# helgeanl/GP-MPC

Measured on NVIDIA H100. Metric: GP predictions/sec (N train x horizon test, fp64), higher is better.
Workload: dtype f64

## Files before the change

gp-mpc_b200/csrc/gpmpc.cu:

```cuda
#include "../../include/gpmpc.h"

#include <dlfcn.h>
#include <math.h>
#include <stdarg.h>
#include <stdlib.h>
#include <string.h>

#include <algorithm>
#include <array>
#include <functional>
#include <map>
#include <memory>
#include <type_traits>
#include <vector>

#include <nvtx3/nvToolsExt.h>

#include "common.cuh"
#include "gemm_dmma.cuh"
#include "predict_streamk.cuh"
#include "kernels.cuh"

#define GPMPC_VERSION 100
#define HB 64
// ... 948 lines not shown
    int used = 0;
    rc = factor_entries(h, e, 1, 1e-8, &used);
    if (rc) return rc;
    if (used > 1) { set_error(h, "gpmpc_loo_nlpp: K not positive definite even with jitter"); return GPMPC_ERR_NOTPD; }
    rc = alpha_pass(h, e);
    if (rc) return rc;
    LooLayout o;
    rc = loo_layout(h, 1, &o);
    if (rc) return rc;
    rc = loo_launch(h, al, 1, o, grad != nullptr);
    if (rc) return rc;
    double val = 0.0;
    CUDA_TRY(cudaMemcpyAsync(&val, o.nlpp, 8, cudaMemcpyDeviceToHost, h->st));
    if (grad) {
        rc = compute_kinv(h, al);
        if (rc) return rc;
        trmv_lower_kernel<<<(N + 7) / 8, 256, 0, h->st>>>(e.Li, np, 0, o.u, 0, o.tmp, 0, N);
        CUDA_TRY(cudaGetLastError());
        trmv_lower_T_kernel<<<(N + 31) / 32, 256, 0, h->st>>>(e.Li, np, 0, o.tmp, 0, o.b, 0, N);
        CUDA_TRY(cudaGetLastError());
        loo_mirror_scale_kernel<<<dim3(np / 32, np / 32), dim3(32, 8), 0, h->st>>>(h->dKinv, np, o.sw, h->dU, N);
        CUDA_TRY(cudaGetLastError());
        GemmParams p;
        memset(&p, 0, sizeof(p));
        p.A = h->dU; p.lda = np; p.B = h->dU; p.ldb = np; p.C = h->dKinv; p.ldc = np;
        p.mt = np / 128; p.nt = np / 128; p.K = np; p.alpha = 1.0; p.beta = 0.0; p.lower = 1;
        CUDA_TRY(gemm128(h, h->st, true, p, 1, 1));
        loo_w_kernel<<<dim3((N + 255) / 256, N), 256, 0, h->st>>>(h->dKinv, np, o.b, e.alpha, N);
        CUDA_TRY(cudaGetLastError());
        CUDA_TRY(cudaMemsetAsync(o.zero, 0, (size_t)np * 8, h->st));
        rc = launch_grad_at(h, e.hyp, h->dKinv, o.zero, h->dGradPart, h->dGrad, 1);
        if (rc) return rc;
        CUDA_TRY(cudaMemcpyAsync(grad, h->dGrad, m * 8, cudaMemcpyDeviceToHost, h->st));
    }
    CUDA_TRY(cudaStreamSynchronize(h->st));
    if (grad)
        for (int q = 0; q < m; ++q) grad[q] *= 2.0;
    *nlpp = val;
    return GPMPC_OK;
}

extern "C" int gpmpc_get(gpmpc_handle_t h, int what, int a, double* dst)
{
    if (!h || !dst) return GPMPC_ERR_ARG;
    CUDA_TRY(cudaSetDevice(h->device));
    const int al = local_index(h, a);
    if (al < 0) return GPMPC_ERR_ARG;
    if (what == GPMPC_GET_K) return gpmpc_build_K(h, a, dst);
    if (what != GPMPC_GET_ALPHA_NLML) {
        const int rc = model_guard(h, __func__, NEED_FACTOR);
        if (rc) return rc;
    }
    switch (what) {
    case GPMPC_GET_CHOL: return extract_to_host(h, h->dL + (long long)al * slab(h), dst, 1);
    case GPMPC_GET_LINV: return extract_to_host(h, h->dLi + (long long)al * slab(h), dst, 1);
    case GPMPC_GET_ALPHA:
    case GPMPC_GET_ALPHA_NLML:
        CUDA_TRY(cudaMemcpyAsync(dst, h->dAlpha + (long long)al * h->Npad, h->N * 8, cudaMemcpyDeviceToHost, h->st));
        CUDA_TRY(cudaStreamSynchronize(h->st));
        return GPMPC_OK;
    case GPMPC_GET_LOGDET: dst[0] = h->logdet[al]; return GPMPC_OK;
    case GPMPC_GET_INVK: {
        int rc = compute_kinv(h, al);
        if (rc) return rc;
        return extract_to_host(h, h->dKinv, dst, 2);
    }
    default: set_error(h, "gpmpc_get: unknown selector %d", what); return GPMPC_ERR_ARG;
    }
}

extern "C" int gpmpc_set_option(gpmpc_handle_t h, const char* name, double value)
{
    if (!h || !name) return GPMPC_ERR_ARG;
    if (!strcmp(name, "refine")) { h->opt_refine = value != 0.0; return GPMPC_OK; }
    if (!strcmp(name, "predict_ctas")) {
        const int v = (int)value;
        if (v < 0 || v > PSK_MAX_CTAS) { set_error(h, "predict_ctas must be in [0, %d]", PSK_MAX_CTAS); return GPMPC_ERR_ARG; }
        h->opt_predict_ctas = v; return GPMPC_OK;
    }
    if (!strcmp(name, "peer_timeout_s")) { h->opt_peer_timeout_s = value > 0.0 ? value : 60.0; return GPMPC_OK; }
    if (!strcmp(name, "small_tiles")) { h->opt_small_tiles = (int)value; return GPMPC_OK; }
    if (!strcmp(name, "peer")) { h->opt_peer = value != 0.0; return GPMPC_OK; }
    if (!strcmp(name, "em_points")) {
        if (!(value >= 0.0 && value <= 1e9)) { set_error(h, "em_points must be >= 0"); return GPMPC_ERR_ARG; }
        h->opt_em_points = (int)value; return GPMPC_OK;
    }
    if (!strcmp(name, "nlml_batch_max")) {
        if (!(value >= 0.0 && value <= 1e9)) { set_error(h, "nlml_batch_max must be >= 0"); return GPMPC_ERR_ARG; }
        h->opt_nlml_batch_max = (int)value; return GPMPC_OK;
    }
    set_error(h, "unknown option %s", name);
    return GPMPC_ERR_ARG;
}

static inline int ks_chunk(gpmpc_handle_t h)
{
    if (h->Npad < 8192) return 128;
    return (h->nloc >= 2 && h->Nx <= 12) ? 1024 : 512;
}

static inline int ks_blocks(gpmpc_handle_t h) { return (h->Npad + ks_chunk(h) - 1) / ks_chunk(h); }

static inline int round8(int n) { return (n + 7) / 8 * 8; }

static int ensure_rows(gpmpc_handle_t h)
{
    ENSURE(h->dV, (long long)h->nloc * HB * h->Npad);
    ENSURE(h->dR, (long long)h->nloc * HB * h->Npad);
    return GPMPC_OK;
}

static int ensure_predict_bufs(gpmpc_handle_t h, int H)
{
    const long long np = h->Npad, nt = np / 128;
    ENSURE(h->dKST, (long long)h->nloc * HB * np);
    ENSURE(h->dPMJ, (long long)h->nloc * HB * ks_blocks(h) * (h->Nx + 1));
    ENSURE(h->dSQ, (long long)h->nloc * HB * nt);
    ENSURE(h->dCnt, (long long)h->nloc * nt + h->nloc + 1);
    ENSURE(h->dPart, (long long)std::max(h->psk_ctas, h->opt_predict_ctas) * 2 * HB * PSK_BN);
    if (h->opt_refine) {
        int rc = ensure_rows(h);
        if (rc) return rc;
        ENSURE(h->dR2, (long long)h->nloc * HB * np);
    }
    if (H > h->Hcap) {
        h->Hcap = 0;
        h->dZ = h->dSigma = h->dMean = h->dVar = h->dJ = h->dCov = nullptr;
        const long long cap = std::max(H, HB);
        const int nyp = h->nloc_max * h->world;
        const long long Nx = h->Nx, Ny = h->Ny;
        ENSURE(h->dG, (long long)nyp * cap * (Nx + 2));
        ENSURE(h->dIn, cap * Nx + cap * Nx * Nx);
        ENSURE(h->dOut, cap * (2 * Ny + Ny * Nx + Ny * Ny));
        h->dZ = h->dIn; h->dSigma = h->dIn + cap * Nx;
        h->dMean = h->dOut; h->dVar = h->dOut + cap * Ny; h->dJ = h->dOut + 2 * cap * Ny;
        h->dCov = h->dOut + 2 * cap * Ny + cap * Ny * Nx;
        h->Hcap = (int)cap;
    }
    return GPMPC_OK;
}

template <int BM>
static cudaError_t psk_launch_bm(const PredictParams& p, const double* A, long long sA, const double* B, long long sB,
                                 int np, int grid, cudaStream_t st)
{
    constexpr int BYTES = psk_pipe_doubles(BM) * 8 + 2 * PSK_STAGES * 8 + 1024;
    const cudaError_t e = smem_opt_in<predict_streamk_kernel<BM>>(BYTES);
    if (e != cudaSuccess) return e;
    CUtensorMap tmA, tmB;
    if (!tmap_make(&tmA, A, np, BM, np, sA, p.nloc, BM)) return cudaErrorInvalidValue;
    if (!tmap_make(&tmB, B, np, np, np, sB, p.nloc, PSK_BN)) return cudaErrorInvalidValue;
    cudaLaunchConfig_t cfg;
    memset(&cfg, 0, sizeof(cfg));
    cfg.gridDim = dim3(grid); cfg.blockDim = dim3(PSK_THREADS); cfg.dynamicSmemBytes = BYTES; cfg.stream = st;
    cudaLaunchAttribute attr[1];
    attr[0].id = cudaLaunchAttributeProgrammaticStreamSerialization;
    attr[0].val.programmaticStreamSerializationAllowed = 1;
    cfg.attrs = attr; cfg.numAttrs = 1;
    return cudaLaunchKernelEx(&cfg, predict_streamk_kernel<BM>, p, tmA, tmB);
}

static int psk_grid(gpmpc_handle_t h, long long G)
{
    int ctas = h->opt_predict_ctas > 0 ? h->opt_predict_ctas : h->psk_ctas;
    ctas = std::min(ctas, PSK_MAX_CTAS);
    const long long by_work = std::max(1LL, G / 4);
    return (int)std::min<long long>(ctas, h->opt_predict_ctas > 0 ? G : by_work);
}

static int psk_schedule(gpmpc_handle_t h, PredictParams& p, const double* B)
{
    int grid = psk_grid(h, p.G);
    if (B == h->dLi.p && !p.upper) {
        p.Lp = h->dLiP;
        p.upo = psk_pair_units(p.nloc, p.ntb, grid);
        if (p.upo && h->opt_predict_ctas == 0) grid = psk_pair_grid((long long)p.nloc * p.upo, grid);
    }
    return grid;
}

static cudaError_t psk_launch(gpmpc_handle_t h, const PredictParams& p0, const double* A, const double* B)
{
    const long long sA = (long long)HB * h->Npad, sB = slab(h);
    const int np = h->Npad;
    PredictParams p = p0;
    const int grid = psk_schedule(h, p, B);
    if (p.Lp)
        for (int a = 0; a < h->nloc; ++a)
            if (h->panel_row[a] < np) return cudaErrorIllegalState;
    switch (round8(p.Hc)) {
    case 8: return psk_launch_bm<8>(p, A, sA, B, sB, np, grid, h->st);
    case 16: return psk_launch_bm<16>(p, A, sA, B, sB, np, grid, h->st);
    case 24: return psk_launch_bm<24>(p, A, sA, B, sB, np, grid, h->st);
    case 32: return psk_launch_bm<32>(p, A, sA, B, sB, np, grid, h->st);
    case 40: return psk_launch_bm<40>(p, A, sA, B, sB, np, grid, h->st);
    case 48: return psk_launch_bm<48>(p, A, sA, B, sB, np, grid, h->st);
    case 56: return psk_launch_bm<56>(p, A, sA, B, sB, np, grid, h->st);
    default: return psk_launch_bm<64>(p, A, sA, B, sB, np, grid, h->st);
    }
}

static void psk_base(gpmpc_handle_t h, PredictParams& p, int Hc, int upper = 0)
{
    memset(&p, 0, sizeof(p));
    const long long nt = h->Npad / 128;
    p.nloc = h->nloc; p.nt = (int)nt; p.Hc = Hc; p.upper = upper;
    p.ntb = (int)((h->Npad + PSK_BN - 1) / PSK_BN); p.nk = h->Npad / GEMM_BK;
    p.T = psk_steps_per_output(p.ntb, p.nk, upper); p.G = p.T * h->nloc;
    p.part = h->dPart;
    p.tile_cnt = h->dCnt; p.out_cnt = h->dCnt + (long long)h->nloc * nt; p.done_cnt = p.out_cnt + h->nloc;
    p.SQ = h->dSQ;
    p.hyp = h->dHyp; p.hyp_ld = h->Nx + 2; p.Nx = h->Nx;
}

static int panel_refresh(gpmpc_handle_t h)
{
    PredictParams p;
    psk_base(h, p, HB);
    const long long blk = PSK_BN * GEMM_BK;
    const double* old = h->dLiP;
    ENSURE(h->dLiP, p.G * blk);
    if (h->dLiP.p != old) panel_stale(h, -1, 0);
    for (int a = 0; a < h->nloc; ++a) {
        if (h->panel_row[a] >= h->Npad) continue;
        const int jt0 = h->panel_row[a] / PSK_BN;
        panel_pack_kernel<<<dim3(p.nk, p.ntb - jt0), 256, 0, h->st>>>(h->dLi + a * slab(h), h->Npad, h->dLiP + a * p.T * blk,
                                                                      p.ntb, jt0);
        CUDA_TRY(cudaGetLastError());
        h->panel_row[a] = h->Npad;
    }
    return GPMPC_OK;
}

static void psk_finalize(gpmpc_handle_t h, PredictParams& p, int H, int h0)
{
    p.finalize = 1; p.PMJ = h->dPMJ; p.nblk_mj = ks_blocks(h);
    p.Gloc = h->dG; p.slot0 = h->a0; p.Htot = H; p.h0 = h0;
}

static AssembleArgs assemble_args(gpmpc_handle_t h, int H, int method, const double* Sigma, int spp,
                                  double* mean, double* var, double* J, double* cov)
{
    AssembleArgs as;
    memset(&as, 0, sizeof(as));
    as.G = h->dG; as.Ny = h->Ny; as.Nx = h->Nx; as.H = H; as.method_ta = (method == GPMPC_METHOD_TA);
    as.Sigma = Sigma; as.sigma_per_point = spp;
    as.mean = mean; as.var = var; as.J = J; as.cov = cov;
    as.world = 1;
    as.stage_g = (assemble_rows_doubles(H, h->Ny, h->Nx) <= psk_pipe_doubles(round8(std::min(H, HB)))) ? 1 : 0;
    return as;
}

template <int NXP, int CH>
static cudaError_t launch_ks(gpmpc_handle_t h, const double* dZc, int Hc)
{
    const int smem = (NXP + 1) * CH * 8, nblk = ks_blocks(h);
    const cudaError_t e = smem_opt_in<ks_tile_kernel<NXP, CH>>(smem);
    if (e != cudaSuccess) return e;
    dim3 g(nblk, round8(Hc) / 8, h->nloc);
    ks_tile_kernel<NXP, CH><<<g, 256, smem, h->st>>>(h->dXT, h->Npad, h->N, h->Nx, h->dHyp, h->Nx + 2, h->dAlpha, h->Npad,
                                                     dZc, Hc, h->dKST, h->Npad, (long long)HB * h->Npad, h->dPMJ, nblk);
    return cudaGetLastError();
}

template <int CH>
static cudaError_t launch_ks_nx(gpmpc_handle_t h, const double* dZc, int Hc)
{
    const int Nx = h->Nx;
    if (Nx <= 4) return launch_ks<4, CH>(h, dZc, Hc);
    if (Nx <= 6) return launch_ks<6, CH>(h, dZc, Hc);
    if (Nx <= 8) return launch_ks<8, CH>(h, dZc, Hc);
    if (Nx <= 10) return launch_ks<10, CH>(h, dZc, Hc);
    if (Nx <= 12) return launch_ks<12, CH>(h, dZc, Hc);
    if (CH <= 512) {
        if (Nx <= 16) return launch_ks<16, (CH <= 512 ? CH : 512)>(h, dZc, Hc);
        if (Nx <= 24) return launch_ks<24, (CH <= 512 ? CH : 512)>(h, dZc, Hc);
        return launch_ks<32, (CH <= 512 ? CH : 512)>(h, dZc, Hc);
    }
    return cudaErrorInvalidValue;
}

static cudaError_t launch_ks(gpmpc_handle_t h, const double* dZc, int Hc)
{
    switch (ks_chunk(h)) {
    case 1024: return launch_ks_nx<1024>(h, dZc, Hc);
    case 512: return launch_ks_nx<512>(h, dZc, Hc);
    default: return launch_ks_nx<128>(h, dZc, Hc);
    }
}

static int tri_product(gpmpc_handle_t h, const double* Amat, const double* T, int Hc, double* Vout)
{
    PredictParams p;
    psk_base(h, p, Hc);
    p.Vout = Vout; p.sV = (long long)HB * h->Npad; p.ldv = h->Npad;
    CUDA_TRY(psk_launch(h, p, Amat, T));
    return GPMPC_OK;
}

__global__ void axpby_rows_kernel(const double* __restrict__ x, const double* __restrict__ y, double a, double b,
                                  double* __restrict__ out, long long rowlen, long long srow, int rows)
{
    const long long i = (long long)blockIdx.x * blockDim.x + threadIdx.x;
    const int r = blockIdx.y, bz = blockIdx.z;
    if (i >= rowlen || r >= rows) return;
    const long long o = (long long)bz * srow + (long long)r * rowlen + i;
    out[o] = a * x[o] + b * y[o];
// ... 2106 lines not shown
```

gp-mpc_b200/csrc/predict_streamk.cuh:

```cuda
#pragma once
#include "common.cuh"
#include "gemm_dmma.cuh"

#define GPMPC_MAXW 16
#define PSK_CW 8
#define PSK_BN (32 * PSK_CW)
#define PSK_STAGES 5
#define PSK_CTAS_PER_SM 1
#define PSK_THREADS (32 * PSK_CW)

__host__ __device__ constexpr long long psk_pipe_doubles(int bm) { return (long long)PSK_STAGES * (bm + PSK_BN) * GEMM_BK; }


struct PeerArgs {
    double* base[GPMPC_MAXW];
    int world, rank;
    long long goff;
    int flag_idx;
    unsigned long long step;
    long long timeout_clocks;
};

struct AssembleArgs {
    const double* G;
    int Ny, Nx, H, method_ta;
    const double* Sigma; int sigma_per_point;
    double *mean, *var, *J, *cov;
    const unsigned long long* flags;
    int world; unsigned long long step; int* status;
    long long timeout_clocks;
    unsigned long long* dbg;
    int stage_g;
};

struct PredictParams {
    int nloc, nt, Hc;
    int ntb, nk;
    int upper;
    const double* Lp;
    long long T, G;
    int upo;
    double* part;
    unsigned int* tile_cnt;
    unsigned int* out_cnt;
    unsigned int* done_cnt;
    double* SQ;
    double* Vout; long long sV; int ldv;
    int finalize;
    const double* PMJ; int nblk_mj;
    const double* hyp; int hyp_ld, Nx;
    double* Gloc; int slot0, Htot, h0;
    PeerArgs pa; int use_peers, publish;
    AssembleArgs as; int do_assemble;
    unsigned long long* dbg;
};

__device__ __forceinline__ void tail_stamp(unsigned long long* dbg, int k, int tid)
{
    if (dbg && tid == 0) { unsigned long long t; asm volatile("mov.u64 %0, %%globaltimer;" : "=l"(t)); dbg[k] = t; }
}

template <bool WARP>
__device__ __forceinline__ void assemble_point(const AssembleArgs& A, int h, double* sh, int tid, int nth)
{
    const int Ny = A.Ny, Nx = A.Nx, H = A.H;
    double* Jh = sh; double* JS = sh + Ny * Nx; double* vh = sh + 2 * Ny * Nx;
    for (int idx = tid; idx < Ny * Nx; idx += nth) {
        const int a = idx / Nx, d = idx % Nx;
        const double v = __ldcg(A.G + (((long long)a) * H + h) * (Nx + 2) + 2 + d);
        Jh[idx] = v;
        if (A.J) A.J[((long long)h * Ny + a) * Nx + d] = v;
    }
    for (int a = tid; a < Ny; a += nth) {
        const double* g = A.G + (((long long)a) * H + h) * (Nx + 2);
        const double m = __ldcg(g), v = __ldcg(g + 1);
        if (A.mean) A.mean[(long long)h * Ny + a] = m;
        if (A.var) A.var[(long long)h * Ny + a] = v;
        vh[a] = v;
    }
    if (WARP) __syncwarp(); else __syncthreads();
    if (A.cov) {
        if (A.method_ta) {
            const double* Sg = A.Sigma + (A.sigma_per_point ? (long long)h * Nx * Nx : 0);
            for (int idx = tid; idx < Ny * Nx; idx += nth) {
                const int a = idx / Nx, e = idx % Nx;
                double s = 0.0;
                for (int d = 0; d < Nx; ++d) s = fma(Jh[a * Nx + d], Sg[d * Nx + e], s);
                JS[idx] = s;
            }
            if (WARP) __syncwarp(); else __syncthreads();
        }
        for (int idx = tid; idx < Ny * Ny; idx += nth) {
            const int a = idx / Ny, b = idx % Ny;
            double s = (a == b) ? vh[a] : 0.0;
            if (A.method_ta) {
                double t = 0.0;
                for (int e = 0; e < Nx; ++e) t = fma(JS[a * Nx + e], Jh[b * Nx + e], t);
                s += t;
            }
            A.cov[((long long)h * Ny + a) * Ny + b] = s;
        }
    }
    if (WARP) __syncwarp(); else __syncthreads();
}

__device__ __forceinline__ void assemble_flat_global(const AssembleArgs& A, double* JS, int tid, int nth)
{
    const int Ny = A.Ny, Nx = A.Nx, H = A.H, NyNx = Ny * Nx;
    const bool ta = A.cov && A.method_ta;
    for (int idx = tid; idx < H * NyNx; idx += nth) {
        const int h = idx / NyNx, r = idx - h * NyNx, a = r / Nx, e = r - a * Nx;
        const double* g = A.G + (((long long)a) * H + h) * (Nx + 2) + 2;
        if (A.J) A.J[idx] = __ldcg(g + e);
        if (ta) {
            const double* Sg = A.Sigma + (A.sigma_per_point ? (long long)h * Nx * Nx : 0);
            double s = 0.0;
            for (int d = 0; d < Nx; ++d) s = fma(__ldcg(g + d), Sg[d * Nx + e], s);
            JS[idx] = s;
        }
    }
    for (int idx = tid; idx < H * Ny; idx += nth) {
        const int h = idx / Ny, a = idx - h * Ny;
        const double* g = A.G + (((long long)a) * H + h) * (Nx + 2);
        if (A.mean) A.mean[idx] = __ldcg(g);
        if (A.var) A.var[idx] = __ldcg(g + 1);
    }
    __syncthreads();
    if (A.cov) {
        for (int idx = tid; idx < H * Ny * Ny; idx += nth) {
            const int h = idx / (Ny * Ny), r = idx - h * Ny * Ny, a = r / Ny, b = r - a * Ny;
            double s = (a == b) ? __ldcg(A.G + (((long long)a) * H + h) * (Nx + 2) + 1) : 0.0;
            if (ta) {
                const double* gb = A.G + (((long long)b) * H + h) * (Nx + 2) + 2;
                const double* js = JS + (h * Ny + a) * Nx;
                double t = 0.0;
                for (int e = 0; e < Nx; ++e) t = fma(js[e], __ldcg(gb + e), t);
                s += t;
            }
            A.cov[idx] = s;
        }
    }
}

__host__ __device__ inline long long assemble_rows_doubles(int H, int Ny, int Nx)
{
    return (long long)H * Ny * (((Nx + 2) | 1) + (Nx | 1)) + (long long)Nx * Nx;
}

__device__ __forceinline__ void assemble_rows(const AssembleArgs& A, double* sh, int tid, int nth)
{
    const int Ny = A.Ny, Nx = A.Nx, H = A.H, F = Nx + 2, FP = F | 1, NP = Nx | 1, R = H * Ny;
    const bool ta = A.cov && A.method_ta;
    double* Gs = sh;
    double* JS = Gs + R * FP;
    double* Ss = JS + R * NP;
    const bool sig_s = ta && !A.sigma_per_point;
    {
        const int tot = R * F, HF = H * F;
        if (sig_s) for (int i = tid; i < Nx * Nx; i += nth) Ss[i] = A.Sigma[i];
        constexpr int SB = 20;
        for (int idx = tid; idx < tot; idx += SB * nth) {
            double v[SB];
#pragma unroll
            for (int k = 0; k < SB; ++k) v[k] = (idx + k * nth < tot) ? __ldcg(A.G + idx + k * nth) : 0.0;
#pragma unroll
            for (int k = 0; k < SB; ++k) {
                const int o = idx + k * nth;
                if (o < tot) {
                    const int a = o / HF, rem = o - a * HF, h = rem / F, q = rem - h * F;
                    Gs[(h * Ny + a) * FP + q] = v[k];
                }
            }
        }
        __syncthreads();
    }
    tail_stamp(A.dbg, 3, tid);
    if (A.J) for (int i = tid; i < R * Nx; i += nth) { const int row = i / Nx; A.J[i] = Gs[row * FP + 2 + (i - row * Nx)]; }
    for (int idx = tid; idx < R; idx += nth) {
        const double* g = Gs + idx * FP;
        if (A.mean) A.mean[idx] = g[0];
        if (A.var) A.var[idx] = g[1];
        if (ta) {
            const int h = idx / Ny;
            const double* Sg = sig_s ? Ss : A.Sigma + (long long)h * Nx * Nx;
            for (int e0 = 0; e0 < Nx; e0 += 8) {
                double acc[8];
#pragma unroll
                for (int k = 0; k < 8; ++k) acc[k] = 0.0;
                for (int d = 0; d < Nx; ++d) {
                    const double jd = g[2 + d];
#pragma unroll
                    for (int k = 0; k < 8; ++k) if (e0 + k < Nx) acc[k] = fma(jd, Sg[d * Nx + e0 + k], acc[k]);
                }
#pragma unroll
                for (int k = 0; k < 8; ++k) if (e0 + k < Nx) JS[idx * NP + e0 + k] = acc[k];
            }
        }
    }
    __syncthreads();
    tail_stamp(A.dbg, 4, tid);
    if (A.cov) {
        const bool via_smem = Ny <= 8 && Ny <= NP;
        for (int idx = tid; idx < R; idx += nth) {
            const int h = idx / Ny, a = idx - h * Ny;
            const double var = Gs[idx * FP + 1];
            for (int b0 = 0; b0 < Ny; b0 += 8) {
                double acc[8];
#pragma unroll
                for (int k = 0; k < 8; ++k) acc[k] = 0.0;
                if (ta) {
                    for (int e = 0; e < Nx; ++e) {
                        const double je = JS[idx * NP + e];
#pragma unroll
                        for (int k = 0; k < 8; ++k) if (b0 + k < Ny) acc[k] = fma(je, Gs[(h * Ny + b0 + k) * FP + 2 + e], acc[k]);
                    }
                }
#pragma unroll
                for (int k = 0; k < 8; ++k) {
                    if (b0 + k < Ny) {
                        const double c = ((a == b0 + k) ? var : 0.0) + acc[k];
                        if (via_smem) JS[idx * NP + k] = c; else A.cov[(long long)idx * Ny + b0 + k] = c;
                    }
                }
            }
        }
        if (via_smem) {
            __syncthreads();
            for (int i = tid; i < R * Ny; i += nth) { const int row = i / Ny; A.cov[i] = JS[row * NP + (i - row * Ny)]; }
        }
    }
}

__device__ __forceinline__ void assemble_flat(const AssembleArgs& A, double* sh, int tid, int nth)
{
    if (A.stage_g) assemble_rows(A, sh, tid, nth);
    else assemble_flat_global(A, sh, tid, nth);
}

__device__ __forceinline__ bool peer_acquire(const AssembleArgs& A, int tid, int* sh_ok)
{
    if (!A.flags) return true;
    if (tid == 0) *sh_ok = 1;
    __syncthreads();
    if (tid < A.world) {
        const long long t0 = clock64();
        unsigned long long v;
        do {
            asm volatile("ld.acquire.sys.global.u64 %0, [%1];" : "=l"(v) : "l"(A.flags + tid) : "memory");
            if (v >= A.step) break;
            if (clock64() - t0 > A.timeout_clocks) {
                *reinterpret_cast<volatile int*>(A.status) = 1 + tid;
                *reinterpret_cast<volatile int*>(sh_ok) = 0;
                break;
            }
            __nanosleep(64);
        } while (true);
    }
    __syncthreads();
    return *reinterpret_cast<volatile int*>(sh_ok) != 0;
}

__global__ void __launch_bounds__(128)
assemble_kernel(const AssembleArgs A)
{
    extern __shared__ double sh[];
    __shared__ int ok;
    if (!peer_acquire(A, threadIdx.x, &ok)) return;
    for (int h = blockIdx.x; h < A.H; h += gridDim.x) assemble_point<false>(A, h, sh, threadIdx.x, blockDim.x);
}

#define PSK_SB (PSK_BN / GEMM_BK)
__host__ __device__ inline long long psk_kstart(int ntb, int nk, int upper, int jt)
{
    const long long full = (long long)(PSK_SB / 2) * jt * (jt + 1), d = (long long)PSK_SB * ntb - nk;
    return upper ? full - jt * d : (jt == ntb ? full - d : full);
}
__host__ __device__ inline long long psk_steps_per_output(int ntb, int nk, int upper) { return psk_kstart(ntb, nk, upper, ntb); }
__device__ __forceinline__ long long psk_kstart(const PredictParams& p, int jt) { return psk_kstart(p.ntb, p.nk, p.upper, jt); }
__host__ __device__ inline int psk_ksteps(int ntb, int nk, int upper, int jt)
{
    return upper ? nk - PSK_SB * (ntb - 1 - jt) : (PSK_SB * (jt + 1) < nk ? PSK_SB * (jt + 1) : nk);
}
__device__ __forceinline__ int psk_ksteps(const PredictParams& p, int jt) { return psk_ksteps(p.ntb, p.nk, p.upper, jt); }

__host__ __device__ inline int psk_pair_units(int nloc, int ntb, int grid)
{
    const long long upo = (ntb + 1) / 2, units = nloc * upo, rounds = (units + grid - 1) / grid;
    return (units >= grid && 8 * units >= 7 * rounds * grid) ? (int)upo : 0;
}
__host__ __device__ inline int psk_pair_grid(long long units, int grid)
{
    const long long rounds = (units + grid - 1) / grid;
    return (int)((units + rounds - 1) / rounds);
}
__host__ __device__ inline int psk_unit_steps(int ntb, int nk, int pu)
{
    const int jl = ntb - 1 - pu;
    return psk_ksteps(ntb, nk, 0, jl) + (pu != jl ? psk_ksteps(ntb, nk, 0, pu) : 0);
}
__host__ __device__ inline long long psk_pair_cta_steps(int nloc, int ntb, int nk, int upo, long long c, long long C)
{
    long long n = 0;
    for (long long u = c; u < (long long)nloc * upo; u += C) n += psk_unit_steps(ntb, nk, (int)(u % upo));
    return n;
}
__host__ __device__ inline void psk_pair_first(int ntb, int upo, long long u, int& a, int& jt)
{
    a = (int)(u / upo);
    jt = ntb - 1 - (int)(u - (long long)a * upo);
}
__host__ __device__ inline void psk_pair_next(int ntb, int upo, long long C, int& a, int& jt)
{
    if (2 * jt > ntb - 1) jt = ntb - 1 - jt;
    else psk_pair_first(ntb, upo, (long long)a * upo + jt + C, a, jt);
}

struct PskIter { int a, jt, s, ks; };

__device__ __forceinline__ void psk_iter_init(PskIter& it, const PredictParams& p, long long c, long long C)
{
    if (p.upo) {
        psk_pair_first(p.ntb, p.upo, c, it.a, it.jt);
        it.s = 0; it.ks = psk_ksteps(p, it.jt);
        return;
    }
    const long long g = p.G * c / C;
    it.a = (int)(g / p.T);
    const long long r = g - (long long)it.a * p.T;
    int jt = (int)((sqrt(8.0 * (double)r / PSK_SB + 1.0) - 1.0) * 0.5);
    jt = max(0, min(jt, p.ntb - 1));
    while (jt > 0 && psk_kstart(p, jt) > r) --jt;
    while (jt + 1 < p.ntb && psk_kstart(p, jt + 1) <= r) ++jt;
    it.jt = jt; it.s = (int)(r - psk_kstart(p, jt)); it.ks = psk_ksteps(p, jt);
}
__device__ __forceinline__ void psk_iter_next(PskIter& it, const PredictParams& p)
{
    if (++it.s == it.ks) {
        it.s = 0;
        if (p.upo) psk_pair_next(p.ntb, p.upo, gridDim.x, it.a, it.jt);
        else if (++it.jt == p.ntb) { it.jt = 0; ++it.a; }
        it.ks = psk_ksteps(p, it.jt);
    }
}

__host__ __device__ inline long long psk_panel_chunk(int ntb, int nk, int jt, int s, int r, int c)
{
    return (psk_kstart(ntb, nk, 0, jt) + s) * (PSK_BN * GEMM_BK) + r * GEMM_BK + 2 * (c ^ (r & 7));
}

__global__ void __launch_bounds__(256)
panel_pack_kernel(const double* __restrict__ Li, int np, double* __restrict__ P, int ntb, int jt0)
{
    const int s = blockIdx.x, jt = jt0 + blockIdx.y, nk = np / GEMM_BK, c = threadIdx.x & 7;
    if (s >= psk_ksteps(ntb, nk, 0, jt)) return;
#pragma unroll 4
    for (int r = threadIdx.x >> 3; r < PSK_BN; r += 32) {
        const long long row = (long long)jt * PSK_BN + r;
        const double2 v = row < np ? __ldcs(reinterpret_cast<const double2*>(Li + row * np + s * GEMM_BK) + c) : make_double2(0.0, 0.0);
        *reinterpret_cast<double2*>(P + psk_panel_chunk(ntb, nk, jt, s, r, c)) = v;
    }
}

__device__ __forceinline__ void psk_store_record(const PredictParams& p, int a, int h, int q, double val)
{
    const long long off = (((long long)(p.slot0 + a)) * p.Htot + p.h0 + h) * (p.Nx + 2) + q;
    if (!p.use_peers) p.Gloc[off] = val;
    else for (int r = 0; r < p.pa.world; ++r) p.pa.base[r][p.pa.goff + off] = val;
}

__device__ __forceinline__ void psk_reduce_mj(const PredictParams& p, int i_begin, int i_end, int t, int nthr)
{
    const int F1 = p.Nx + 1;
    for (int i = i_begin + t; i < i_end; i += nthr) {
        const int ah = i / F1, qq = i - ah * F1, a = ah / p.Hc, h = ah - a * p.Hc;
        const double* pm = p.PMJ + ((long long)ah * p.nblk_mj) * F1 + qq;
        double s0 = 0.0, s1 = 0.0;
        int b = 0;
        for (; b + 16 <= p.nblk_mj; b += 16) {
            double v[16];
#pragma unroll
            for (int k = 0; k < 16; ++k) v[k] = __ldcg(pm + (long long)(b + k) * F1);
#pragma unroll
            for (int k = 0; k < 16; k += 2) { s0 += v[k]; s1 += v[k + 1]; }
        }
        for (; b + 2 <= p.nblk_mj; b += 2) { s0 += __ldcg(pm + (long long)b * F1); s1 += __ldcg(pm + (long long)(b + 1) * F1); }
        if (b < p.nblk_mj) s0 += __ldcg(pm + (long long)b * F1);
        psk_store_record(p, a, h, qq == 0 ? 0 : qq + 1, s0 + s1);
    }
}

__device__ __forceinline__ void psk_finalize_output(const PredictParams& p, int a, int tid, int nth)
{
    const int Nx = p.Nx;
    const double sf = p.hyp[(long long)a * p.hyp_ld + Nx];
    for (int base = 0; base < p.Hc; base += nth / 4) {
        const int h = base + (tid >> 2), j0 = tid & 3;
        double sj = 0.0;
        if (h < p.Hc) {
            const double* sq = p.SQ + ((long long)a * 64 + h) * p.nt;
            int j = j0;
            for (; j + 4 * 15 < p.nt; j += 4 * 16) {
                double v[16];
#pragma unroll
                for (int k = 0; k < 16; ++k) v[k] = __ldcg(sq + j + 4 * k);
#pragma unroll
                for (int k = 0; k < 16; ++k) sj += v[k];
            }
            for (; j < p.nt; j += 4) sj += __ldcg(sq + j);
        }
        sj += __shfl_xor_sync(0xffffffffu, sj, 1);
        sj += __shfl_xor_sync(0xffffffffu, sj, 2);
        if (h < p.Hc && j0 == 0) psk_store_record(p, a, h, 1, sf * sf - sj);
    }
    if (p.use_peers) __threadfence_system(); else __threadfence();
}

__device__ __forceinline__ void psk_step_tail(const PredictParams& p, double* sh, int tid, int nth,
                                              unsigned int* s_flag, int* s_ok)
{
    __syncthreads();
    if (tid == 0) {
        const unsigned int old = atomicAdd(p.done_cnt, 1u);
        const unsigned int last = (old == (unsigned int)(p.nloc - 1)) ? 1u : 0u;
        if (last) *p.done_cnt = 0u;
        *s_flag = last;
    }
    __syncthreads();
    if (*s_flag == 0u) return;
    if (p.finalize && p.use_peers && p.publish && tid == 0) {
        __threadfence_system();
        for (int r = 0; r < p.pa.world; ++r) {
            unsigned long long* f = reinterpret_cast<unsigned long long*>(p.pa.base[r]) + p.pa.flag_idx;
            asm volatile("st.release.sys.global.u64 [%0], %1;" :: "l"(f), "l"(p.pa.step) : "memory");
        }
    }
    tail_stamp(p.as.dbg, 2, tid);
    if (p.do_assemble) {
        __threadfence();
        if (peer_acquire(p.as, tid, s_ok)) assemble_flat(p.as, sh, tid, nth);
    }
    __syncthreads();
    tail_stamp(p.as.dbg, 5, tid);
}

__global__ void __launch_bounds__(128)
sq_rows_kernel(const double* __restrict__ V, int ldv, long long sV, double* __restrict__ SQ, int nt)
{
    __shared__ double red[4];
    const int jt = blockIdx.x, h = blockIdx.y, a = blockIdx.z;
    const double v = V[(long long)a * sV + (long long)h * ldv + jt * 128 + threadIdx.x];
    const double s = warp_sum(v * v);
    if ((threadIdx.x & 31) == 0) red[threadIdx.x >> 5] = s;
    __syncthreads();
    if (threadIdx.x == 0) SQ[((long long)a * 64 + h) * nt + jt] = (red[0] + red[1]) + (red[2] + red[3]);
}

__global__ void __launch_bounds__(PSK_THREADS)
finalize_kernel(const PredictParams p)
{
    extern __shared__ double sh[];
    __shared__ unsigned int s_flag;
    __shared__ int s_ok;
    const int per = p.Hc * (p.Nx + 1);
    psk_reduce_mj(p, blockIdx.x * per, (blockIdx.x + 1) * per, threadIdx.x, PSK_THREADS);
    psk_finalize_output(p, blockIdx.x, threadIdx.x, PSK_THREADS);
    psk_step_tail(p, sh, threadIdx.x, PSK_THREADS, &s_flag, &s_ok);
}

template <int BM>
__global__ void __launch_bounds__(PSK_THREADS, PSK_CTAS_PER_SM)
predict_streamk_kernel(const PredictParams p, const __grid_constant__ CUtensorMap tmA, const __grid_constant__ CUtensorMap tmB)
{
    constexpr int BK = GEMM_BK, BN = PSK_BN, STAGES = PSK_STAGES, CW = PSK_CW, NT = PSK_THREADS;
    constexpr int NF = BM / 8;
    static_assert(BK == 16 && BN == 32 * CW && BN % 128 == 0, "one m16n8k16 per fragment and k-step, 32 L-rows per warp");
    constexpr int GR = BN / 128;
    constexpr int A_STAGE = BM * BK, B_STAGE = BN * BK;
    constexpr uint32_t STAGE_TX = (BM + BN) * BK * 8;
    static_assert(BM % 8 == 0 && BM >= 8 && BM <= 64, "BM");

    extern __shared__ __align__(16) double smem_raw[];
    double* smem = smem_align1024(smem_raw);
    double* As = smem;
    double* Bs = smem + STAGES * A_STAGE;
    uint64_t* full = reinterpret_cast<uint64_t*>(smem + STAGES * (A_STAGE + B_STAGE));
    uint64_t* empty = full + STAGES;
    __shared__ double red[BN / 16][64];
    __shared__ unsigned int s_flag;
    __shared__ int s_ok;

    const int tid = threadIdx.x, warp = tid >> 5, lane = tid & 31, g = lane >> 2, t = lane & 3;
    const long long C = gridDim.x, c = blockIdx.x;
    const int nsteps = p.upo ? (int)psk_pair_cta_steps(p.nloc, p.ntb, p.nk, p.upo, c, C)
                             : (int)(p.G * (c + 1) / C - p.G * c / C);
    if (nsteps <= 0) return;
    if (p.dbg && threadIdx.x == 0) { unsigned long long t0; asm volatile("mov.u64 %0, %%globaltimer;" : "=l"(t0)); p.dbg[2 * blockIdx.x] = t0; }

    __shared__ PskIter s_pit;
    __shared__ int s_pg;
    __shared__ uint64_t s_pol[2];
    if (tid == 0) {
#pragma unroll
        for (int s = 0; s < STAGES; ++s) { mbar_init(full + s, 1); mbar_init(empty + s, CW); }
        mbar_fence_init();
    }
    __syncthreads();

    auto issue = [&]() {
        PskIter it = s_pit;
        const int pg = s_pg, s = pg % STAGES;
        if (pg >= STAGES) mbar_wait(empty + s, (uint32_t)(((pg / STAGES) - 1) & 1));
        mbar_arrive_expect_tx(full + s, STAGE_TX);
        const int jta = p.upper ? p.ntb - 1 - it.jt : it.jt;
        const int k0 = (p.upper ? jta * BN : 0) + it.s * BK;
        tma_tile_g2s_3d_hint(As + s * A_STAGE, &tmA, k0, 0, it.a, full + s, s_pol[1]);
        if (p.Lp) bulk_g2s_hint(Bs + s * B_STAGE, p.Lp + ((long long)it.a * p.T + psk_kstart(p, it.jt) + it.s) * B_STAGE,
                                B_STAGE * 8, full + s, s_pol[0]);
        else tma_tile_g2s_3d_hint(Bs + s * B_STAGE, &tmB, k0, jta * BN, it.a, full + s, s_pol[0]);
        psk_iter_next(it, p);
        s_pit = it;
        s_pg = pg + 1;
    };
    constexpr int AHEAD = STAGES - 2;
    asm volatile("griddepcontrol.wait;" ::: "memory");
    if (tid == 0) {
        PskIter it;
        psk_iter_init(it, p, c, C);
        s_pit = it; s_pg = 0;
        s_pol[0] = l2_policy_evict_first(); s_pol[1] = l2_policy_evict_last();
#pragma unroll
        for (int s = 0; s < AHEAD; ++s)
            if (s_pg < nsteps) issue();
    }
    if (p.finalize) {
        const int tot = p.nloc * p.Hc * (p.Nx + 1), per = (tot + (int)C - 1) / (int)C;
        if (tid >= 32) {
            psk_reduce_mj(p, min(tot, (int)c * per), min(tot, ((int)c + 1) * per), tid - 32, NT - 32);
            if (p.use_peers) __threadfence_system();
        }
    }

    PskIter cit;
    psk_iter_init(cit, p, c, C);
    int cj[4];
#pragma unroll
    for (int j = 0; j < 4; ++j) cj[j] = (((j + 4 * (t >> 1)) ^ g) << 1) + (t & 1);
    int i = 0;
    while (i < nsteps) {
        const int a = cit.a, jt = cit.jt, s_begin = cit.s, ksteps = cit.ks;
        const int seg = min(ksteps - s_begin, nsteps - i);
        const int hh = warp / (128 / 32);
        const int st_lo = p.upper ? (128 / BK) * hh : 0;
        const int st_hi = p.upper ? ksteps : PSK_SB * jt + (128 / BK) * (hh + 1);
        double acc[2][NF][4];
#pragma unroll
        for (int mi = 0; mi < 2; ++mi)
#pragma unroll
            for (int ni = 0; ni < NF; ++ni)
#pragma unroll
                for (int r = 0; r < 4; ++r) acc[mi][ni][r] = 0.0;

        for (int q = 0; q < seg; ++q, ++i) {
            const int s = i % STAGES;
            if (tid == 0 && i + AHEAD < nsteps) issue();
            mbar_wait(full + s, (uint32_t)((i / STAGES) & 1));
            const int st = s_begin + q;
            if (st >= st_lo && st < st_hi) {
                const double* ls = Bs + s * B_STAGE + (warp * 32 + g) * 16;
                const double* ps = As + s * A_STAGE + g * 16;
                double av[2][8];
#pragma unroll
                for (int mi = 0; mi < 2; ++mi)
#pragma unroll
                    for (int j = 0; j < 4; ++j) { av[mi][2 * j] = ls[256 * mi + cj[j]]; av[mi][2 * j + 1] = ls[256 * mi + 128 + cj[j]]; }
#pragma unroll
                for (int ni = 0; ni < NF; ++ni) {
                    double bv[4];
#pragma unroll
                    for (int j = 0; j < 4; ++j) bv[j] = ps[ni * 8 * 16 + cj[j]];
                    dmma16816(acc[0][ni], av[0], bv);
                    dmma16816(acc[1][ni], av[1], bv);
                }
            }
            __syncwarp();
            if (lane == 0) mbar_arrive(empty + s);
        }
        cit.s = s_begin + seg - 1;
        psk_iter_next(cit, p);

        bool have_tile = true;
        if (seg != ksteps) {
            const long long tg0 = (long long)a * p.T + psk_kstart(p, jt), tg1 = tg0 + ksteps;
            const long long Cf = gridDim.x;
            const int c_first = (int)(((tg0 + 1) * Cf - 1) / p.G), c_last = (int)((tg1 * Cf - 1) / p.G);
            double2* mine = reinterpret_cast<double2*>(p.part + ((long long)blockIdx.x * 2 + (s_begin == 0 ? 1 : 0)) * (BM * BN)) + tid;
#pragma unroll
            for (int mi = 0; mi < 2; ++mi)
#pragma unroll
                for (int ni = 0; ni < NF; ++ni)
#pragma unroll
                    for (int hf = 0; hf < 2; ++hf)
                        __stcg(mine + ((mi * NF + ni) * 2 + hf) * NT, make_double2(acc[mi][ni][2 * hf], acc[mi][ni][2 * hf + 1]));
            __threadfence();
            __syncthreads();
            if (tid == 0) {
                unsigned int* cnt = p.tile_cnt + (long long)a * p.ntb + jt;
                const unsigned int old = atomicAdd(cnt, 1u);
                const unsigned int last = (old == (unsigned int)(c_last - c_first)) ? 1u : 0u;
                if (last) *cnt = 0u;
                s_flag = last;
            }
            __syncthreads();
            have_tile = s_flag != 0u;
            if (have_tile) {
                __threadfence();
#pragma unroll
                for (int mi = 0; mi < 2; ++mi)
#pragma unroll
                    for (int ni = 0; ni < NF; ++ni)
#pragma unroll
                        for (int r = 0; r < 4; ++r) acc[mi][ni][r] = 0.0;
                for (int cc = c_first; cc <= c_last; ++cc) {
                    const double2* src = reinterpret_cast<const double2*>(p.part + ((long long)cc * 2 + (cc == c_first ? 1 : 0)) * (BM * BN)) + tid;
#pragma unroll
                    for (int mi = 0; mi < 2; ++mi)
#pragma unroll
                        for (int ni = 0; ni < NF; ++ni)
#pragma unroll
                            for (int hf = 0; hf < 2; ++hf) {
                                const double2 v = __ldcg(src + ((mi * NF + ni) * 2 + hf) * NT);
                                acc[mi][ni][2 * hf] += v.x; acc[mi][ni][2 * hf + 1] += v.y;
                            }
                }
            }
        }
        if (!have_tile) continue;

        const int jta = p.upper ? p.ntb - 1 - jt : jt;
        const int row0 = jta * BN + warp * 32;
        if (p.Vout && row0 < p.nk * BK) {
            double* vo = p.Vout + (long long)a * p.sV + row0 + g;
#pragma unroll
            for (int mi = 0; mi < 2; ++mi)
#pragma unroll
                for (int ni = 0; ni < NF; ++ni)
#pragma unroll
                    for (int r = 0; r < 4; ++r)
                        vo[(long long)(ni * 8 + 2 * t + (r & 1)) * p.ldv + 16 * mi + 8 * (r >> 1)] = acc[mi][ni][r];
        }
#pragma unroll
        for (int mi = 0; mi < 2; ++mi)
#pragma unroll
            for (int ni = 0; ni < NF; ++ni)
#pragma unroll
                for (int j = 0; j < 2; ++j) {
                    double r = acc[mi][ni][j] * acc[mi][ni][j];
                    r = fma(acc[mi][ni][j + 2], acc[mi][ni][j + 2], r);
                    r += __shfl_xor_sync(0xffffffffu, r, 4);
                    r += __shfl_xor_sync(0xffffffffu, r, 8);
                    r += __shfl_xor_sync(0xffffffffu, r, 16);
                    if (g == 0) red[2 * warp + mi][ni * 8 + 2 * t + j] = r;
                }
        __syncthreads();
        for (int idx = tid; idx < GR * BM; idx += NT) {
            const int gr = idx / BM, pt = idx - gr * BM, col = jta * GR + gr;
            if (col < p.nt) {
                double r = 0.0;
#pragma unroll
                for (int b = 0; b < 8; ++b) r += red[8 * gr + b][pt];
                __stcg(p.SQ + ((long long)a * 64 + pt) * p.nt + col, r);
            }
        }
        __threadfence();
        __syncthreads();
        if (tid == 0) {
            unsigned int* cnt = p.out_cnt + a;
            const unsigned int old = atomicAdd(cnt, 1u);
            const unsigned int last = (old == (unsigned int)(p.ntb - 1)) ? 1u : 0u;
            if (last) *cnt = 0u;
            s_flag = last;
        }
        __syncthreads();
        if (s_flag == 0u) continue;

        __threadfence();
        tail_stamp(p.as.dbg, 0, tid);
        if (p.finalize) psk_finalize_output(p, a, tid, NT);
        tail_stamp(p.as.dbg, 1, tid);
        psk_step_tail(p, smem, tid, NT, &s_flag, &s_ok);
    }
    if (p.dbg && threadIdx.x == 0) { unsigned long long t1; asm volatile("mov.u64 %0, %%globaltimer;" : "=l"(t1)); p.dbg[2 * blockIdx.x + 1] = t1; }
}
```

Measured before the change: 16860.

## Warp-specialize stream-K predict kernel with dedicated TMA producer warpgroup and setmaxnreg

Adds a 128-thread producer warpgroup to the stream-K predict kernel. One thread issues all TMA loads for the whole step range, and the other three warps run the finalize reduction. The consumer warps drop in-loop TMA issue and rebalance registers via setmaxnreg, and block-wide syncs become named barriers over consumer threads only. The goal is to take load issue off the MMA critical path and deepen prefetch beyond the old AHEAD=3. The cost is extra named-barrier coordination and a risky register split. The bar 2 handshake also looks fragile: it only triggers on the first segment and only for warp 0, with a count of 128.

```diff
diff --git a/gp-mpc_b200/csrc/gpmpc.cu b/gp-mpc_b200/csrc/gpmpc.cu
--- a/gp-mpc_b200/csrc/gpmpc.cu
+++ b/gp-mpc_b200/csrc/gpmpc.cu
@@ -1124,7 +1124,7 @@
     if (!tmap_make(&tmB, B, np, np, np, sB, p.nloc, PSK_BN)) return cudaErrorInvalidValue;
     cudaLaunchConfig_t cfg;
     memset(&cfg, 0, sizeof(cfg));
-    cfg.gridDim = dim3(grid); cfg.blockDim = dim3(PSK_THREADS); cfg.dynamicSmemBytes = BYTES; cfg.stream = st;
+    cfg.gridDim = dim3(grid); cfg.blockDim = dim3(PSK_LAUNCH_THREADS); cfg.dynamicSmemBytes = BYTES; cfg.stream = st;
     cudaLaunchAttribute attr[1];
     attr[0].id = cudaLaunchAttributeProgrammaticStreamSerialization;
     attr[0].val.programmaticStreamSerializationAllowed = 1;
diff --git a/gp-mpc_b200/csrc/predict_streamk.cuh b/gp-mpc_b200/csrc/predict_streamk.cuh
--- a/gp-mpc_b200/csrc/predict_streamk.cuh
+++ b/gp-mpc_b200/csrc/predict_streamk.cuh
@@ -8,6 +8,11 @@
 #define PSK_STAGES 5
 #define PSK_CTAS_PER_SM 1
 #define PSK_THREADS (32 * PSK_CW)
+#define PSK_LAUNCH_THREADS (128 + PSK_THREADS)
+#define PSK_PRODUCER_REGS 40
+#define PSK_CONSUMER_REGS 232
+
+__device__ __forceinline__ void psk_sync(int nth) { asm volatile("bar.sync 1, %0;" :: "r"(nth) : "memory"); }
 
 __host__ __device__ constexpr long long psk_pipe_doubles(int bm) { return (long long)PSK_STAGES * (bm + PSK_BN) * GEMM_BK; }
 
@@ -125,7 +130,7 @@
         if (A.mean) A.mean[idx] = __ldcg(g);
         if (A.var) A.var[idx] = __ldcg(g + 1);
     }
-    __syncthreads();
+    psk_sync(nth);
     if (A.cov) {
         for (int idx = tid; idx < H * Ny * Ny; idx += nth) {
             const int h = idx / (Ny * Ny), r = idx - h * Ny * Ny, a = r / Ny, b = r - a * Ny;
@@ -172,7 +177,7 @@
                 }
             }
         }
-        __syncthreads();
+        psk_sync(nth);
     }
     tail_stamp(A.dbg, 3, tid);
     if (A.J) for (int i = tid; i < R * Nx; i += nth) { const int row = i / Nx; A.J[i] = Gs[row * FP + 2 + (i - row * Nx)]; }
@@ -197,7 +202,7 @@
             }
         }
     }
-    __syncthreads();
+    psk_sync(nth);
     tail_stamp(A.dbg, 4, tid);
     if (A.cov) {
         const bool via_smem = Ny <= 8 && Ny <= NP;
@@ -225,7 +230,7 @@
             }
         }
         if (via_smem) {
-            __syncthreads();
+            psk_sync(nth);
             for (int i = tid; i < R * Ny; i += nth) { const int row = i / Ny; A.cov[i] = JS[row * NP + (i - row * Ny)]; }
         }
     }
@@ -237,11 +242,11 @@
     else assemble_flat_global(A, sh, tid, nth);
 }
 
-__device__ __forceinline__ bool peer_acquire(const AssembleArgs& A, int tid, int* sh_ok)
+__device__ __forceinline__ bool peer_acquire(const AssembleArgs& A, int tid, int nth, int* sh_ok)
 {
     if (!A.flags) return true;
     if (tid == 0) *sh_ok = 1;
-    __syncthreads();
+    psk_sync(nth);
     if (tid < A.world) {
         const long long t0 = clock64();
         unsigned long long v;
@@ -256,7 +261,7 @@
             __nanosleep(64);
         } while (true);
     }
-    __syncthreads();
+    psk_sync(nth);
     return *reinterpret_cast<volatile int*>(sh_ok) != 0;
 }
 
@@ -265,7 +270,7 @@
 {
     extern __shared__ double sh[];
     __shared__ int ok;
-    if (!peer_acquire(A, threadIdx.x, &ok)) return;
+    if (!peer_acquire(A, threadIdx.x, blockDim.x, &ok)) return;
     for (int h = blockIdx.x; h < A.H; h += gridDim.x) assemble_point<false>(A, h, sh, threadIdx.x, blockDim.x);
 }
 
@@ -306,8 +311,8 @@
 }
 __host__ __device__ inline void psk_pair_first(int ntb, int upo, long long u, int& a, int& jt)
 {
-    a = (int)(u / upo);
-    jt = ntb - 1 - (int)(u - (long long)a * upo);
+    a = (int)u / upo;
+    jt = ntb - 1 - ((int)u - a * upo);
 }
 __host__ __device__ inline void psk_pair_next(int ntb, int upo, long long C, int& a, int& jt)
 {
@@ -418,14 +423,14 @@
 __device__ __forceinline__ void psk_step_tail(const PredictParams& p, double* sh, int tid, int nth,
                                               unsigned int* s_flag, int* s_ok)
 {
-    __syncthreads();
+    psk_sync(nth);
     if (tid == 0) {
         const unsigned int old = atomicAdd(p.done_cnt, 1u);
         const unsigned int last = (old == (unsigned int)(p.nloc - 1)) ? 1u : 0u;
         if (last) *p.done_cnt = 0u;
         *s_flag = last;
     }
-    __syncthreads();
+    psk_sync(nth);
     if (*s_flag == 0u) return;
     if (p.finalize && p.use_peers && p.publish && tid == 0) {
         __threadfence_system();
@@ -437,9 +442,9 @@
     tail_stamp(p.as.dbg, 2, tid);
     if (p.do_assemble) {
         __threadfence();
-        if (peer_acquire(p.as, tid, s_ok)) assemble_flat(p.as, sh, tid, nth);
-    }
-    __syncthreads();
+        if (peer_acquire(p.as, tid, nth, s_ok)) assemble_flat(p.as, sh, tid, nth);
+    }
+    psk_sync(nth);
     tail_stamp(p.as.dbg, 5, tid);
 }
 
@@ -468,12 +473,13 @@
 }
 
 template <int BM>
-__global__ void __launch_bounds__(PSK_THREADS, PSK_CTAS_PER_SM)
+__global__ void __launch_bounds__(PSK_LAUNCH_THREADS, PSK_CTAS_PER_SM)
 predict_streamk_kernel(const PredictParams p, const __grid_constant__ CUtensorMap tmA, const __grid_constant__ CUtensorMap tmB)
 {
     constexpr int BK = GEMM_BK, BN = PSK_BN, STAGES = PSK_STAGES, CW = PSK_CW, NT = PSK_THREADS;
     constexpr int NF = BM / 8;
     static_assert(BK == 16 && BN == 32 * CW && BN % 128 == 0, "one m16n8k16 per fragment and k-step, 32 L-rows per warp");
+    static_assert(128 * PSK_PRODUCER_REGS + NT * PSK_CONSUMER_REGS <= 168 * PSK_LAUNCH_THREADS, "setmaxnreg split of the register file");
     constexpr int GR = BN / 128;
     constexpr int A_STAGE = BM * BK, B_STAGE = BN * BK;
     constexpr uint32_t STAGE_TX = (BM + BN) * BK * 8;
@@ -489,59 +495,62 @@
     __shared__ unsigned int s_flag;
     __shared__ int s_ok;
 
-    const int tid = threadIdx.x, warp = tid >> 5, lane = tid & 31, g = lane >> 2, t = lane & 3;
-    const long long C = gridDim.x, c = blockIdx.x;
-    const int nsteps = p.upo ? (int)psk_pair_cta_steps(p.nloc, p.ntb, p.nk, p.upo, c, C)
-                             : (int)(p.G * (c + 1) / C - p.G * c / C);
-    if (nsteps <= 0) return;
-    if (p.dbg && threadIdx.x == 0) { unsigned long long t0; asm volatile("mov.u64 %0, %%globaltimer;" : "=l"(t0)); p.dbg[2 * blockIdx.x] = t0; }
-
-    __shared__ PskIter s_pit;
-    __shared__ int s_pg;
-    __shared__ uint64_t s_pol[2];
-    if (tid == 0) {
+    __shared__ PskIter s_it0;
+    __shared__ int s_nsteps;
+    if (threadIdx.x == 0) {
 #pragma unroll
         for (int s = 0; s < STAGES; ++s) { mbar_init(full + s, 1); mbar_init(empty + s, CW); }
         mbar_fence_init();
     }
     __syncthreads();
 
-    auto issue = [&]() {
-        PskIter it = s_pit;
-        const int pg = s_pg, s = pg % STAGES;
-        if (pg >= STAGES) mbar_wait(empty + s, (uint32_t)(((pg / STAGES) - 1) & 1));
-        mbar_arrive_expect_tx(full + s, STAGE_TX);
-        const int jta = p.upper ? p.ntb - 1 - it.jt : it.jt;
-        const int k0 = (p.upper ? jta * BN : 0) + it.s * BK;
-        tma_tile_g2s_3d_hint(As + s * A_STAGE, &tmA, k0, 0, it.a, full + s, s_pol[1]);
-        if (p.Lp) bulk_g2s_hint(Bs + s * B_STAGE, p.Lp + ((long long)it.a * p.T + psk_kstart(p, it.jt) + it.s) * B_STAGE,
-                                B_STAGE * 8, full + s, s_pol[0]);
-        else tma_tile_g2s_3d_hint(Bs + s * B_STAGE, &tmB, k0, jta * BN, it.a, full + s, s_pol[0]);
-        psk_iter_next(it, p);
-        s_pit = it;
-        s_pg = pg + 1;
-    };
-    constexpr int AHEAD = STAGES - 2;
+    if (threadIdx.x < 128) {
+        asm volatile("setmaxnreg.dec.sync.aligned.u32 %0;" :: "n"(PSK_PRODUCER_REGS));
+        asm volatile("griddepcontrol.wait;" ::: "memory");
+        if (threadIdx.x < 32) asm volatile("bar.sync 3, %0;" :: "n"(NT + 32) : "memory");
+        if (threadIdx.x == 0 && s_nsteps > 0) {
+            if (p.dbg) { unsigned long long t0; asm volatile("mov.u64 %0, %%globaltimer;" : "=l"(t0)); p.dbg[2 * blockIdx.x] = t0; }
+            const uint64_t pol_a = l2_policy_evict_last(), pol_b = l2_policy_evict_first();
+            PskIter it = s_it0;
+            const int nsteps = s_nsteps;
+            for (int pg = 0; pg < nsteps; ++pg) {
+                const int s = pg % STAGES;
+                if (pg >= STAGES) mbar_wait(empty + s, (uint32_t)(((pg / STAGES) - 1) & 1));
+                mbar_arrive_expect_tx(full + s, STAGE_TX);
+                const int jta = p.upper ? p.ntb - 1 - it.jt : it.jt;
+                const int k0 = (p.upper ? jta * BN : 0) + it.s * BK;
+                tma_tile_g2s_3d_hint(As + s * A_STAGE, &tmA, k0, 0, it.a, full + s, pol_a);
+                if (p.Lp) bulk_g2s_hint(Bs + s * B_STAGE, p.Lp + ((long long)it.a * p.T + psk_kstart(p, it.jt) + it.s) * B_STAGE,
+                                        B_STAGE * 8, full + s, pol_b);
+                else tma_tile_g2s_3d_hint(Bs + s * B_STAGE, &tmB, k0, jta * BN, it.a, full + s, pol_b);
+                psk_iter_next(it, p);
+            }
+        } else if (threadIdx.x >= 32) {
+            if (p.finalize) {
+                const int tot = p.nloc * p.Hc * (p.Nx + 1), per = (tot + (int)gridDim.x - 1) / (int)gridDim.x, c = blockIdx.x;
+                psk_reduce_mj(p, min(tot, c * per), min(tot, (c + 1) * per), threadIdx.x - 32, 96);
+                if (p.use_peers) __threadfence_system();
+            }
+            asm volatile("bar.arrive 2, 128;" ::: "memory");
+        }
+        return;
+    }
+
+    asm volatile("setmaxnreg.inc.sync.aligned.u32 %0;" :: "n"(PSK_CONSUMER_REGS));
     asm volatile("griddepcontrol.wait;" ::: "memory");
+    const int tid = threadIdx.x - 128, warp = tid >> 5, lane = tid & 31, g = lane >> 2, t = lane & 3;
     if (tid == 0) {
+        const long long C = gridDim.x, c = blockIdx.x;
+        s_nsteps = p.upo ? (int)psk_pair_cta_steps(p.nloc, p.ntb, p.nk, p.upo, c, C)
+                         : (int)(p.G * (c + 1) / C - p.G * c / C);
         PskIter it;
         psk_iter_init(it, p, c, C);
-        s_pit = it; s_pg = 0;
-        s_pol[0] = l2_policy_evict_first(); s_pol[1] = l2_policy_evict_last();
-#pragma unroll
-        for (int s = 0; s < AHEAD; ++s)
-            if (s_pg < nsteps) issue();
-    }
-    if (p.finalize) {
-        const int tot = p.nloc * p.Hc * (p.Nx + 1), per = (tot + (int)C - 1) / (int)C;
-        if (tid >= 32) {
-            psk_reduce_mj(p, min(tot, (int)c * per), min(tot, ((int)c + 1) * per), tid - 32, NT - 32);
-            if (p.use_peers) __threadfence_system();
-        }
-    }
-
-    PskIter cit;
-    psk_iter_init(cit, p, c, C);
+        s_it0 = it;
+    }
+    asm volatile("bar.sync 3, %0;" :: "n"(NT + 32) : "memory");
+    const int nsteps = s_nsteps;
+    if (nsteps <= 0) return;
+    PskIter cit = s_it0;
     int cj[4];
 #pragma unroll
     for (int j = 0; j < 4; ++j) cj[j] = (((j + 4 * (t >> 1)) ^ g) << 1) + (t & 1);
@@ -562,7 +571,6 @@
 
         for (int q = 0; q < seg; ++q, ++i) {
             const int s = i % STAGES;
-            if (tid == 0 && i + AHEAD < nsteps) issue();
             mbar_wait(full + s, (uint32_t)((i / STAGES) & 1));
             const int st = s_begin + q;
             if (st >= st_lo && st < st_hi) {
@@ -587,6 +595,7 @@
         }
         cit.s = s_begin + seg - 1;
         psk_iter_next(cit, p);
+        if (i == seg && warp == 0) asm volatile("bar.sync 2, 128;" ::: "memory");
 
         bool have_tile = true;
         if (seg != ksteps) {
@@ -602,7 +611,7 @@
                     for (int hf = 0; hf < 2; ++hf)
                         __stcg(mine + ((mi * NF + ni) * 2 + hf) * NT, make_double2(acc[mi][ni][2 * hf], acc[mi][ni][2 * hf + 1]));
             __threadfence();
-            __syncthreads();
+            psk_sync(NT);
             if (tid == 0) {
                 unsigned int* cnt = p.tile_cnt + (long long)a * p.ntb + jt;
                 const unsigned int old = atomicAdd(cnt, 1u);
@@ -610,7 +619,7 @@
                 if (last) *cnt = 0u;
                 s_flag = last;
             }
-            __syncthreads();
+            psk_sync(NT);
             have_tile = s_flag != 0u;
             if (have_tile) {
                 __threadfence();
@@ -661,7 +670,7 @@
                     r += __shfl_xor_sync(0xffffffffu, r, 16);
                     if (g == 0) red[2 * warp + mi][ni * 8 + 2 * t + j] = r;
                 }
-        __syncthreads();
+        psk_sync(NT);
         for (int idx = tid; idx < GR * BM; idx += NT) {
             const int gr = idx / BM, pt = idx - gr * BM, col = jta * GR + gr;
             if (col < p.nt) {
@@ -672,7 +681,7 @@
             }
         }
         __threadfence();
-        __syncthreads();
+        psk_sync(NT);
         if (tid == 0) {
             unsigned int* cnt = p.out_cnt + a;
             const unsigned int old = atomicAdd(cnt, 1u);
@@ -680,7 +689,7 @@
             if (last) *cnt = 0u;
             s_flag = last;
         }
-        __syncthreads();
+        psk_sync(NT);
         if (s_flag == 0u) continue;
 
         __threadfence();
@@ -689,5 +698,5 @@
         tail_stamp(p.as.dbg, 1, tid);
         psk_step_tail(p, smem, tid, NT, &s_flag, &s_ok);
     }
-    if (p.dbg && threadIdx.x == 0) { unsigned long long t1; asm volatile("mov.u64 %0, %%globaltimer;" : "=l"(t1)); p.dbg[2 * blockIdx.x + 1] = t1; }
-}
+    if (p.dbg && tid == 0) { unsigned long long t1; asm volatile("mov.u64 %0, %%globaltimer;" : "=l"(t1)); p.dbg[2 * blockIdx.x + 1] = t1; }
+}
```

New measurement: 16880 (median of 6 runs). Within noise of the previous version (+0.2%).
